# lia2790/walking-controllers

Measured on AMD Instinct MI355X. Metric: QP solves/sec (whole node), iCub IK-QP + DCM-MPC batch at 1/2/4/8 MI355X, higher is better.
Workload: dtype f64

## Files before the change

### include/wcqp.h

```cpp
#ifndef WCQP_H
#define WCQP_H

#include <stdint.h>

#ifdef __cplusplus
extern "C" {
#endif

#define WCQP_VERSION 400

#define WCQP_OK              0
#define WCQP_E_INVALID      (-1)
#define WCQP_E_UNSUPPORTED  (-2)
#define WCQP_E_NUMERIC      (-3)
#define WCQP_E_HIP          (-4)
#define WCQP_E_NOMEM        (-5)

#define WCQP_STATUS_SOLVED        0
#define WCQP_STATUS_MAX_ITER      1
#define WCQP_STATUS_INFEASIBLE    2
#define WCQP_STATUS_OUTSIDE_HULL  3
#define WCQP_STATUS_NUMERIC       4
#define WCQP_STATUS_STRUCTURE     5

// ... 101 lines not shown
                       double* foot_err, int32_t* iters);

typedef struct wcqp_qp_step {
    const double* x0; const double* ref; int32_t ref_len; const double* u_prev;
    const double* hull_A; const double* hull_b; const int32_t* hull_nc;
    double* u0; int32_t* mpc_status; uint32_t* mpc_active; double* mpc_margin; void* mpc_stream;
    const double* J_left; const double* J_right; const double* J_neck; const double* J_com;
    const double* q; const double* state;
    double* dq; int32_t* ik_status; uint32_t* active_lower; uint32_t* active_upper;
    double* foot_err; int32_t* iters; void* ik_stream;
} wcqp_qp_step;
int wcqp_qp_enqueue_steps(wcqp_mpc_t mpc, wcqp_ik_t ik, int32_t batch,
                          int32_t n_steps, const wcqp_qp_step* steps, int32_t* n_done);

#define WCQP_PLAN_WAYS_AUTO (-1)
typedef struct wcqp_qp_plan_s* wcqp_qp_plan_t;
int wcqp_qp_plan_create(wcqp_mpc_t mpc, wcqp_ik_t ik, int32_t batch, int32_t n_steps, const wcqp_qp_step* steps, int32_t ways,
                        wcqp_qp_plan_t* out);
int wcqp_qp_plan_enqueue(wcqp_qp_plan_t plan, void* stream);
int wcqp_qp_plan_destroy(wcqp_qp_plan_t plan);

#define WCQP_SLAB_IN_ARRAYS  12
#define WCQP_SLAB_OUT_ARRAYS 9
typedef struct wcqp_slab_layout {
    int32_t batch, ref_len;
    int64_t in_offset[WCQP_SLAB_IN_ARRAYS];
    int64_t in_bytes;
    int64_t out_offset[WCQP_SLAB_OUT_ARRAYS];
    int64_t out_bytes;
} wcqp_slab_layout;
int wcqp_slab_layout_for(int32_t batch, int32_t ref_len, wcqp_slab_layout* out);
int wcqp_qp_step_from_slabs(const wcqp_slab_layout* layout, const void* in_slab, void* out_slab, wcqp_qp_step* step);

#define WCQP_KIN_MAX_DOF 32
// ... 302 lines not shown
```

### walking-controllers_amd/capi.py

```python
from __future__ import annotations

import ctypes as C
import os
from typing import Optional

import numpy as np

_HERE = os.path.dirname(os.path.abspath(__file__))
LIB_PATH = os.environ.get("WCQP_LIB_PATH") or os.path.join(_HERE, "libwcqp.so")

VERSION = 400
WCQP_OK = OK = 0
E_INVALID, E_UNSUPPORTED, E_NUMERIC, E_HIP, E_NOMEM = -1, -2, -3, -4, -5
STATUS_SOLVED, STATUS_MAX_ITER, STATUS_INFEASIBLE, STATUS_OUTSIDE_HULL, STATUS_NUMERIC, STATUS_STRUCTURE = range(6)
IK_FORM_QPOASES, IK_FORM_OSQP = 0, 1
IK_ALG_DEFAULT, IK_ALG_SWEEP, IK_ALG_NULLSPACE, IK_ALG_NULLSPACE_MFMA, IK_ALG_NULLSPACE_16L, IK_ALG_BASE_ELIM = 0, 1, 2, 3, 4, 5
IK_JAC_AUTO, IK_JAC_MIXED, IK_JAC_GENERAL = 0, 1, 2
KIN_HANDOFF_NONE, KIN_HANDOFF_FUSED, KIN_HANDOFF_DENSE, KIN_HANDOFF_COMPACT = -1, 0, 1, 2
HULL_ROWS = 8
MAX_DOF = KIN_MAX_DOF = 32
IK_STATE_LEN = 87

ABI_SYMBOLS = (
    "wcqp_strerror", "wcqp_version", "wcqp_device_count", "wcqp_stream_create", "wcqp_stream_destroy", "wcqp_stream_synchronize",
    "wcqp_mpc_create", "wcqp_mpc_destroy", "wcqp_mpc_get_condensed", "wcqp_mpc_get_matrices",
    "wcqp_mpc_solve_device", "wcqp_mpc_solve_host",
    "wcqp_ik_create", "wcqp_ik_destroy", "wcqp_ik_set_posture", "wcqp_ik_solve_device", "wcqp_ik_solve_host",
    "wcqp_hull_from_feet_device", "wcqp_hull_from_feet_host",
    "wcqp_kin_create", "wcqp_kin_destroy", "wcqp_kin_jacobians_device", "wcqp_kin_jacobians_host",
    "wcqp_prepare_create", "wcqp_prepare_destroy", "wcqp_prepare_solve_device", "wcqp_prepare_solve_host",
    "wcqp_tick_create", "wcqp_tick_create_ext", "wcqp_tick_create_opts", "wcqp_tick_get_option", "wcqp_tick_get_info_ext", "wcqp_tick_destroy", "wcqp_tick_upload", "wcqp_tick_run", "wcqp_tick_download", "wcqp_tick_splice_reference",
    "wcqp_tick_set_feedback_device", "wcqp_tick_set_feedback_host", "wcqp_tick_get_info",
    "wcqp_tick_set_sensor_feedback_device", "wcqp_tick_set_sensor_feedback_host",
    "wcqp_tick_set_desired_device", "wcqp_tick_set_desired_host", "wcqp_tick_set_desired_from_plan",
    "wcqp_tick_upload_footsteps", "wcqp_tick_upload_footsteps_timed", "wcqp_tick_replan_footsteps_timed", "wcqp_tick_get_plan", "wcqp_tick_replan_footsteps", "wcqp_tick_replan_goals", "wcqp_tick_get_goal_result",
    "wcqp_tick_replan_goals_timed", "wcqp_tick_get_goal_timing",
    "wcqp_qp_enqueue_steps", "wcqp_qp_plan_create", "wcqp_qp_plan_enqueue", "wcqp_qp_plan_destroy",
    "wcqp_slab_layout_for", "wcqp_qp_step_from_slabs",
    "wcqp_unicycle_create", "wcqp_unicycle_destroy", "wcqp_unicycle_plan_device", "wcqp_unicycle_plan_host",
    "wcqp_unicycle_plan_timed_device", "wcqp_unicycle_plan_timed_host",
)


class WcqpError(RuntimeError):
    pass


class MpcParams(C.Structure):
    _fields_ = [("horizon", C.c_int32), ("sampling_time", C.c_double), ("com_height", C.c_double),
                ("gravity", C.c_double), ("Q", C.c_double * 4), ("R", C.c_double * 4),
                ("convex_hull_tolerance", C.c_double), ("feas_tol", C.c_double)]

# ... 66 lines not shown
class _Handle:

    def close(self):
        if self._h:
            getattr(lib(), self._destroy)(self._h)
            self._h = C.c_void_p()

    def __del__(self):
        try:
            self.close()
        except Exception:
            pass


PLAN_WAYS_AUTO = -1


class QpPlan(_Handle):
    _destroy = "wcqp_qp_plan_destroy"

    def __init__(self, mpc, ik, batch, steps, ways=1):
        self._h = C.c_void_p()
        self._keep = (mpc, ik, steps)
        check(lib().wcqp_qp_plan_create(mpc._h if mpc is not None else None, ik._h if ik is not None else None, int(batch), len(steps), steps, int(ways), C.byref(self._h)), "wcqp_qp_plan_create")

    def enqueue(self, stream=0):
        check(lib().wcqp_qp_plan_enqueue(self._h, stream or None), "wcqp_qp_plan_enqueue")


class KinParams(C.Structure):
    _fields_ = [("dof", C.c_int32), ("parent", C.c_int32 * 32),
                ("R0", (C.c_double * 9) * 32), ("p0", (C.c_double * 3) * 32), ("axis", (C.c_double * 3) * 32),
                ("mass", C.c_double * 32), ("com", (C.c_double * 3) * 32),
                ("root_mass", C.c_double), ("root_com", C.c_double * 3),
                ("frame_joint", C.c_int32 * 3), ("frame_R", (C.c_double * 9) * 3), ("frame_p", (C.c_double * 3) * 3)]


class PrepareParams(C.Structure):
    _fields_ = [("w_q", C.c_double), ("w_n", C.c_double), ("step_cap", C.c_double), ("tol_step", C.c_double), ("tol_constraint", C.c_double),
                ("max_iter", C.c_int32), ("q_reg", C.c_void_p), ("q_min", C.c_void_p), ("q_max", C.c_void_p)]


# ... 122 lines not shown


ABI_STRUCTS = {
    "wcqp_mpc_params": MpcParams, "wcqp_ik_params": IkParams, "wcqp_qp_step": QpStep, "wcqp_slab_layout": SlabLayout, "wcqp_kin_params": KinParams,
    "wcqp_prepare_params": PrepareParams, "wcqp_tick_params": TickParams, "wcqp_tick_params_ext": TickParamsExt, "wcqp_tick_option": TickOption,
    "wcqp_tick_inputs": TickInputs, "wcqp_tick_outputs": TickOutputs, "wcqp_tick_info": TickInfo, "wcqp_tick_info_ext": TickInfoExt,
    "wcqp_tick_desired": TickDesired, "wcqp_tick_footsteps": TickFootsteps, "wcqp_tick_replan": TickReplan, "wcqp_tick_plan_window": TickPlanWindow,
    "wcqp_tick_goals": TickGoals, "wcqp_tick_goal_result": TickGoalResult, "wcqp_tick_step_timing": TickStepTiming,
    "wcqp_unicycle_params": UnicycleParams, "wcqp_unicycle_inputs": UnicycleInputs, "wcqp_unicycle_outputs": UnicycleOutputs,
    "wcqp_unicycle_timing": UnicycleTiming,
}
ABI_CONSTANTS = {"WCQP_" + k: globals()[k] for k in (
    "VERSION OK E_INVALID E_UNSUPPORTED E_NUMERIC E_HIP E_NOMEM "
    "STATUS_SOLVED STATUS_MAX_ITER STATUS_INFEASIBLE STATUS_OUTSIDE_HULL STATUS_NUMERIC STATUS_STRUCTURE HULL_ROWS MAX_DOF IK_STATE_LEN "
    "IK_FORM_QPOASES IK_FORM_OSQP IK_ALG_DEFAULT IK_ALG_SWEEP IK_ALG_NULLSPACE IK_ALG_NULLSPACE_MFMA IK_ALG_NULLSPACE_16L IK_ALG_BASE_ELIM "
    "IK_JAC_AUTO IK_JAC_MIXED IK_JAC_GENERAL PLAN_WAYS_AUTO SLAB_IN_ARRAYS SLAB_OUT_ARRAYS KIN_MAX_DOF "
    "KIN_HANDOFF_FUSED KIN_HANDOFF_DENSE KIN_HANDOFF_COMPACT TICK_PLANT_INTERNAL TICK_PLANT_EXTERNAL TICK_DCM_MPC TICK_DCM_REACTIVE "
    "TICK_IK_VELOCITY TICK_IK_POSITION TICK_OPT_RESIDENT_PLAN TICK_OPT_POSITION_STREAMED TICK_OPT_PLAN_TIMED UNICYCLE_DONE UNICYCLE_TRUNCATED UNICYCLE_STUCK UNICYCLE_INVALID_INPUT "
    "TICK_MERGE_KEEP TICK_MERGE_AUTO TICK_SIDE_AUTO GOAL_KEPT GOAL_TOO_LATE").split()}

_lib: Optional[C.CDLL] = None


def lib() -> C.CDLL:
    global _lib
    if _lib is None:
        if not os.path.exists(LIB_PATH):
            raise WcqpError(f"{LIB_PATH} is missing: build it with __graft_entry__.build() "
                            "(make -C walking-controllers_amd/csrc); there is no fallback path")
        L = C.CDLL(LIB_PATH)
        dp, ip, up, vp = C.c_void_p, C.c_void_p, C.c_void_p, C.c_void_p
# ... 51 lines not shown
        L.wcqp_tick_replan_goals.argtypes = [C.c_void_p, C.c_void_p, C.POINTER(TickGoals), C.c_void_p]
        L.wcqp_tick_get_goal_result.argtypes = [C.c_void_p, C.POINTER(TickGoalResult)]
        L.wcqp_tick_replan_goals_timed.argtypes = [C.c_void_p, C.c_void_p, C.POINTER(UnicycleTiming), C.POINTER(TickGoals), C.c_void_p]
        L.wcqp_tick_get_goal_timing.argtypes = [C.c_void_p, C.c_void_p, C.c_void_p]
        L.wcqp_unicycle_create.argtypes = [C.POINTER(UnicycleParams), C.POINTER(C.c_void_p)]
        L.wcqp_unicycle_destroy.argtypes = [C.c_void_p]
        L.wcqp_unicycle_plan_device.argtypes = [C.c_void_p, C.c_int32, C.POINTER(UnicycleInputs), C.POINTER(UnicycleOutputs), C.c_void_p]
        L.wcqp_unicycle_plan_host.argtypes = [C.c_void_p, C.c_int32, C.POINTER(UnicycleInputs), C.POINTER(UnicycleOutputs)]
        L.wcqp_unicycle_plan_timed_device.argtypes = [C.c_void_p, C.POINTER(UnicycleTiming), C.c_int32, C.POINTER(UnicycleInputs), C.POINTER(UnicycleOutputs),
                                                      C.c_void_p, C.c_void_p, C.c_void_p]
        L.wcqp_unicycle_plan_timed_host.argtypes = [C.c_void_p, C.POINTER(UnicycleTiming), C.c_int32, C.POINTER(UnicycleInputs), C.POINTER(UnicycleOutputs),
                                                    C.c_void_p, C.c_void_p]
        L.wcqp_qp_enqueue_steps.argtypes = [C.c_void_p, C.c_void_p, C.c_int32, C.c_int32, C.POINTER(QpStep), C.POINTER(C.c_int32)]
        L.wcqp_qp_plan_create.argtypes = [C.c_void_p, C.c_void_p, C.c_int32, C.c_int32, C.POINTER(QpStep), C.c_int32, C.POINTER(C.c_void_p)]
        L.wcqp_qp_plan_enqueue.argtypes = [C.c_void_p, C.c_void_p]
        L.wcqp_qp_plan_destroy.argtypes = [C.c_void_p]
        L.wcqp_slab_layout_for.argtypes = [C.c_int32, C.c_int32, C.POINTER(SlabLayout)]
        L.wcqp_qp_step_from_slabs.argtypes = [C.POINTER(SlabLayout), C.c_void_p, C.c_void_p, C.POINTER(QpStep)]
        _lib = L
    return _lib


def check(rc: int, what: str = "wcqp call") -> None:
    if rc != WCQP_OK:
        raise WcqpError(f"{what} failed: {lib().wcqp_strerror(rc).decode()} ({rc})")


def _p(a: Optional[np.ndarray]):
    return None if a is None else a.ctypes.data_as(C.c_void_p)

# ... 712 lines not shown
```

### walking-controllers_amd/csrc/ik.hip

```cpp
#include <cmath>
#include <cstring>
#include <limits>
#include <new>
#include "ik_common.h"

using namespace wcqp_ik;
#ifdef WCQP_DIAG_KERNELS
#include "../../tools/diag/ik_sweep_kernel.h"
#endif

struct wcqp_ik_s {
    wcqp_ik_params p{};
    IkDeviceParams hp{};
    IkDeviceParams* d_prm = nullptr;
    wcqp::DeviceScratch scratch;
    wcqp::IkRoute route = wcqp::IkRoute::NULLSPACE_32;
    bool list_pass = false;
};

namespace {

int ensure_device(wcqp_ik_s* h) {
    if (h->d_prm) return WCQP_OK;
    if (const int rc = wcqp::require_device("IK solve path"); rc != WCQP_OK) return rc;
// ... 166 lines not shown
    if (!s.J_right || !s.J_neck || !s.J_com || !s.q || !s.state || !s.dq || !s.ik_status) return WCQP_E_INVALID;
    int rc = ensure_device(h);
    if (rc != WCQP_OK) return rc;
    rc = mpc_prepare(mpc);
    if (rc != WCQP_OK) return rc;
    wcqp_mpc::MpcDeviceConsts c;
    mpc_device_consts(mpc, &c);
    const wcqp_ik::IkIo io{s.J_left, s.J_right, s.J_neck, s.J_com, s.q, s.state, s.dq, s.ik_status, s.active_lower, s.active_upper, s.foot_err, s.iters};
    const hipStream_t st = (hipStream_t)s.ik_stream;
    rc = wcqp_ik::ik4_launch_pair(h->d_prm, batch, io, c, s.x0, s.ref, s.ref_len, s.u_prev, s.hull_A, s.hull_b, s.hull_nc,
                                  s.u0, s.mpc_status, s.mpc_active, s.mpc_margin, st);
    return rc != WCQP_OK || !h->list_pass ? rc : wcqp_ik::ik3_launch_list(h->d_prm, batch, io, st);
}
}

struct wcqp_qp_plan_s {
    wcqp_mpc_t mpc = nullptr;
    wcqp_ik_t ik = nullptr;
    int batch = 0, n_steps = 0, ways = 1;
    wcqp_qp_step* d_recs = nullptr;
    unsigned* d_queue = nullptr;
    int queue_grid = 0;
    bool mpc_only = false;
    bool ik_only = false;
};

extern "C" {

int wcqp_qp_plan_create(wcqp_mpc_t mpc, wcqp_ik_t ik, int32_t batch, int32_t n_steps, const wcqp_qp_step* steps, int32_t ways,
                        wcqp_qp_plan_t* out) {
    if (!out || batch < 1 || n_steps < 1 || !steps || ways < WCQP_PLAN_WAYS_AUTO) return WCQP_E_INVALID;
    if (ways == WCQP_PLAN_WAYS_AUTO) {
        const int groups = (batch + 3) / 4;
        ways = (16384 + groups - 1) / groups;
        if (ways < 4) ways = 4;
        if (ways > n_steps) ways = n_steps;
    }
    bool mpc_only = true;
    for (int k = 0; k < n_steps; ++k) mpc_only = mpc_only && !steps[k].J_left;
    bool ik_only = true;
// ... 15 lines not shown
    int rc = mpc_only ? WCQP_OK : ensure_device(ik);
    if (rc == WCQP_OK && mpc) rc = wcqp::mpc_prepare(mpc);
    if (rc != WCQP_OK) return rc;
    wcqp_qp_plan_s* p = new (std::nothrow) wcqp_qp_plan_s();
    if (!p) return WCQP_E_NOMEM;
    p->mpc = mpc; p->ik = mpc_only ? nullptr : ik; p->batch = batch; p->n_steps = n_steps; p->ways = ways < n_steps ? ways : n_steps;
    p->mpc_only = mpc_only; p->ik_only = ik_only;
    if (hipMalloc(reinterpret_cast<void**>(&p->d_recs), (size_t)n_steps * sizeof(wcqp_qp_step)) != hipSuccess) { delete p; return WCQP_E_NOMEM; }
    if (hipMemcpy(p->d_recs, steps, (size_t)n_steps * sizeof(wcqp_qp_step), hipMemcpyHostToDevice) != hipSuccess) {
        (void)hipFree(p->d_recs); delete p; return WCQP_E_HIP;
    }
    if (ways == 0) {
        p->queue_grid = wcqp_ik::ik4_plan_queue_grid(batch, n_steps);
        if (p->queue_grid < 1 || hipMalloc(reinterpret_cast<void**>(&p->d_queue), wcqp_ik::kPlanQueueBytes) != hipSuccess ||
            hipMemset(p->d_queue, 0, wcqp_ik::kPlanQueueBytes) != hipSuccess) {
            if (p->d_queue) (void)hipFree(p->d_queue);
            (void)hipFree(p->d_recs); delete p; return WCQP_E_HIP;
        }
        (void)hipStreamSynchronize(nullptr);
    }
    *out = p;
    return WCQP_OK;
}

int wcqp_qp_plan_enqueue(wcqp_qp_plan_t p, void* stream) {
    if (!p) return WCQP_E_INVALID;
    if (p->mpc_only) return wcqp::mpc_launch_plan(p->mpc, p->batch, p->d_recs, p->n_steps, p->ways, (hipStream_t)stream);
    wcqp_mpc::MpcDeviceConsts c{};
    if (p->mpc) wcqp::mpc_device_consts(p->mpc, &c);
    return wcqp_ik::ik4_launch_plan(p->ik->d_prm, p->batch, p->d_recs, p->n_steps, p->ways, c, (hipStream_t)stream, p->d_queue, p->queue_grid, p->ik_only);
}

int wcqp_qp_plan_destroy(wcqp_qp_plan_t p) {
    if (!p) return WCQP_E_INVALID;
    if (p->d_recs) (void)hipFree(p->d_recs);
    if (p->d_queue) (void)hipFree(p->d_queue);
    delete p;
    return WCQP_OK;
}

}

extern "C" {

int wcqp_ik_solve_host(wcqp_ik_t h, int32_t batch,
                       const double* J_left, const double* J_right, const double* J_neck, const double* J_com,
                       const double* q, const double* state,
                       double* dq, int32_t* status, uint32_t* active_lower, uint32_t* active_upper,
                       double* foot_err, int32_t* iters) {
    int rc = check_call(h, batch, J_left, J_right, J_neck, J_com, q, state, dq, status);
    if (rc != WCQP_OK || batch == 0) return rc;
    rc = ensure_device(h);
// ... 18 lines not shown
```

### walking-controllers_amd/csrc/ik4.hip

```cpp
#include "ik4_device.h"

namespace {

template <bool TICK, int JSRC, bool LOG = false, bool EXT = false>
__global__ __launch_bounds__(64, WCQP_IK4_WAVES)
void ik4_kernel(const IkDeviceParams* __restrict__ prm, int batch,
                const double* __restrict__ JL, const double* __restrict__ JR,
                const double* __restrict__ JN, const double* __restrict__ JC,
                const double* qpos, const double* __restrict__ state,
                double* __restrict__ dq_out, int* __restrict__ status_out,
                unsigned* __restrict__ alo_out, unsigned* __restrict__ aup_out,
                double* __restrict__ ferr_out, int* __restrict__ iters_out, const wcqp_tick::TickDev* __restrict__ tdp, int phase, int n_inner, int skip_last_mpc)
{
    __shared__ __attribute__((aligned(16))) double smem[4][PER_INST];
    if constexpr (TICK) {
        __shared__ __attribute__((aligned(16))) double kmodel[JSRC == 2 ? wcqp_tick::kKinTabSize : 2];
        __shared__ __attribute__((aligned(16))) double kgains[JSRC == 2 ? 4 * wcqp_tick::kGainsLdsStages : 2];
        ik4_tick_walk<JSRC, LOG, EXT, false>(prm, batch, JL, JR, JN, JC, qpos, state, dq_out, status_out, alo_out, aup_out, ferr_out, iters_out,
                                             tdp, phase, n_inner, skip_last_mpc, smem, kmodel, kgains);
    } else {
        ik4_body<TICK, JSRC>(prm, batch, JL, JR, JN, JC, qpos, state, dq_out, status_out, alo_out, aup_out, ferr_out, iters_out, wcqp_tick::TickDev{}, smem, xcd_group((int)blockIdx.x, (int)gridDim.x));
    }
}

// ... 71 lines not shown
            const unsigned u = (unsigned)__builtin_amdgcn_readfirstlane((int)k) * wcqp_ik::kPlanQueues + home;
            if (u < total) return u;
            home = (home + 1u) % wcqp_ik::kPlanQueues;
        }
        return total;
    };
    int r = (int)blockIdx.x / groups, blk = (int)blockIdx.x % groups;
#ifndef WCQP_PLAN_NO_XCD_MAP
    if ((groups & 7) == 0) {
        const int n = groups >> 3, x = (int)blockIdx.x & 7, k = (int)blockIdx.x >> 3;
        r = k / n; blk = x * n + k % n;
    }
#endif
    PlanTables pt;
    plan_tables_issue<TAB>(prm, c, WITH_MPC, ptab, pt);
    if (dynamic) {
        const unsigned u = draw();
        r = u < total ? (int)(u % (unsigned)n_steps) : n_steps; blk = u < total ? (int)(u / (unsigned)n_steps) : 0;
    }
#pragma unroll 1
    while (r < n_steps) {
        __asm__ volatile("" ::: "memory");
        using wcqp::as_global;
        const wcqp_qp_step& s = recs[r];
        MpcPairArgs m{c, WITH_MPC ? as_global(s.x0) : nullptr, WITH_MPC ? as_global(s.ref) : nullptr, s.ref_len, WITH_MPC ? as_global(s.u_prev) : nullptr,
                      WITH_MPC ? as_global(s.hull_A) : nullptr, WITH_MPC ? as_global(s.hull_b) : nullptr, WITH_MPC ? as_global(s.hull_nc) : nullptr,
                      WITH_MPC ? as_global(s.u0) : nullptr, WITH_MPC ? as_global(s.mpc_status) : nullptr, WITH_MPC ? as_global(s.mpc_active) : nullptr,
                      WITH_MPC ? as_global(s.mpc_margin) : nullptr,
                      dynamic ? queue + home * QS + z : nullptr, 0u, WITH_MPC};
        ik4_body<false, 0, true, false, false, false, false, false, TAB>(prm, batch, as_global(s.J_left), as_global(s.J_right), as_global(s.J_neck), as_global(s.J_com), as_global(s.q), as_global(s.state),
                                 as_global(s.dq), as_global(s.ik_status), as_global(s.active_lower), as_global(s.active_upper),
                                 as_global(s.foot_err), as_global(s.iters), wcqp_tick::TickDev{}, smem, blk, 0, true, nullptr, nullptr, &m, nullptr, nullptr, nullptr, &pt);
        wcqp::wave_lds_fence();
        pt.fill = false; pt.f_ik[0] = pt.f_ik[1] = pt.f_ik[2] = 0.0; pt.f_gr[0] = pt.f_gr[1] = make_double2(0.0, 0.0);
        if (dynamic) {
            unsigned u = (unsigned)__builtin_amdgcn_readfirstlane((int)m.ticket) * wcqp_ik::kPlanQueues + home;
            if (u >= total) { home = (home + 1u) % wcqp_ik::kPlanQueues; u = draw(); }
            r = u < total ? (int)(u % (unsigned)n_steps) : n_steps; blk = u < total ? (int)(u / (unsigned)n_steps) : 0;
        } else {
            r += ways;
        }
    }
    if (dynamic && threadIdx.x == 0) {
        __threadfence();
        if (atomicAdd(queue + wcqp_ik::kPlanQueues * QS, 1u) == gridDim.x - 1) {
            for (unsigned q = 0; q <= wcqp_ik::kPlanQueues; ++q) queue[q * QS] = 0u;
        }
    }
}
// ... 107 lines not shown
```

### walking-controllers_amd/csrc/ik4_device.h

```cpp
#pragma once
#include <cmath>
#include <cstddef>
#include <limits>
#include <type_traits>
#include "ik_common.h"
#include "tick_device.h"
#include "kin_device.h"
#include "ik4_layout.h"

namespace {

using wcqp_kin::st2;
using wcqp_kin::ld2;

struct MpcPairArgs {
    wcqp_mpc::MpcDeviceConsts c;
    const double* x0; const double* ref; int ref_len; const double* u_prev;
    const double* hull_A; const double* hull_b; const int* hull_nc;
    double* u0; int* status; unsigned* active; double* margin;
    unsigned* ticket_from = nullptr; unsigned ticket = 0;
    bool has_mpc = true;
};

#ifndef WCQP_PLAN_LDS
// ... 594 lines not shown
        {
            double* c = ct + j * LDC;
#pragma unroll
            for (int r = 0; r < NR; r += 2) st2(c + r, c0[r], c0[r + 1]);
            st2(c + NR, gt0, 0.0);
        }
        if (j < 8) {
            double* c = ct + col1 * LDC;
#pragma unroll
            for (int r = 0; r < NR; r += 2) st2(c + r, rhs1 ? 0.0 : c1[r], rhs1 ? 0.0 : c1[r + 1]);
            st2(c + NR, gt1, 0.0);
        }
        if (rhs1) {
#pragma unroll
            for (int r = 0; r < NR; r += 2) st2(dv + r, c1[r], c1[r + 1]);
            ct[24 * LDC] = 0.0; ct[24 * LDC + 1] = 0.0;
        }
    }
    wcqp::wave_lds_fence();
    WCQP_STAMP(10);
    {
        const int mk = lane & 15, mq = lane >> 4;
        v4d acc[4];
#pragma unroll
        for (int g = 0; g < 4; ++g) acc[g] = v4d{0.0, 0.0, 0.0, 0.0};
#pragma unroll
        for (int s = 0; s < 6; ++s) {
#pragma unroll
            for (int g = 0; g < 4; ++g) {
                const double v = smem[g][OFF_CT + (4 * s + mq) * LDC + mk];
                acc[g] = __builtin_amdgcn_mfma_f64_16x16x4f64(v, v, acc[g], 0, 0, 0);
// ... 775 lines not shown
```

### walking-controllers_amd/csrc/ik4_layout.h

```cpp
#pragma once
#include "ik_common.h"

namespace {

using namespace wcqp_ik;

typedef double v4d __attribute__((ext_vector_type(4)));

constexpr int NR = 12;
constexpr int NROWS_IN = 18;
constexpr int KMAX = kDof - 9;
constexpr int LDC = 14;

constexpr int OFF_ST = 0;
constexpr int OFF_BV = 112;
constexpr int OFF_DB = 130;
constexpr int OFF_CT = 0;
constexpr int OFF_PB = 0;
constexpr int A_SIZE = 340;
constexpr int OFF_COL = A_SIZE;
constexpr int OFF_YV = A_SIZE + 32;
constexpr int OFF_DV = A_SIZE + 48;
constexpr int OFF_YPV = A_SIZE;
constexpr int OFF_RV = A_SIZE + 16;
// ... 2 lines not shown
constexpr int PER_INST = 440;
constexpr int K_FS = 14, K_TW = 0, K_FRB = 322, K_FR = 358;
constexpr int K_MS = 394, K_MH = 410;
constexpr int K_PF = 434;
__host__ __device__ constexpr int k_sd(int m) { return K_TW + (16 + (m >> 1)) * K_FS + 12 + (m & 1); }
static_assert(K_MH + 24 <= K_PF && K_PF < PER_INST, "the flags stash is clear of the others");
static_assert(kDof * K_FS <= K_FRB && K_FR + 36 <= K_MS && K_MH + 24 <= PER_INST && k_sd(11) < kDof * K_FS && k_sd(0) >= 32 * 4, "kinematics scratch fits; the prefix sums [32][4] stay clear of the anchor pose");
static_assert(OFF_CT + 24 * LDC + 2 <= A_SIZE && OFF_DB + 18 <= A_SIZE && OFF_PB + 12 * 18 <= A_SIZE, "LDS overlays");
static_assert(OFF_ROWB + 16 <= PER_INST && OFF_DV + 16 <= PER_INST && (PER_INST % 32 == 24 || PER_INST % 32 == 8), "instances 16 banks apart");
static_assert(KMAX <= 24, "one slot index per C^T row");
static_assert(PER_INST * 8 * 4 * 11 <= 160 * 1024, "11 blocks per CU");

#ifndef WCQP_IK4_WAVES
#define WCQP_IK4_WAVES 2
#endif
#ifdef WCQP_IK_PLAN_VGPR_HALF
#define WCQP_IK_PLAN_REGS __attribute__((amdgpu_num_vgpr(WCQP_IK_PLAN_VGPR_HALF)))
#else
#define WCQP_IK_PLAN_REGS
#endif
#ifndef WCQP_IK4_KS
#define WCQP_IK4_KS 4
#endif

#define WCQP_STAMP_CLOCK(t__) asm volatile("s_memtime %0\n\ts_waitcnt lgkmcnt(0)" : "=s"(t__) :: "memory")
#define WCQP_STAMP_AT(k) do { if constexpr (TICK) { unsigned long long t__; WCQP_STAMP_CLOCK(t__); \
                                   if (lane == 0 && td.stamps) td.stamps[(size_t)blk * 16 + (k)] = t__; } } while (0)
#if defined(WCQP_TICK_KSTAMPS)
#define WCQP_STAMP(k) do { if constexpr ((k) == 0 || (k) == 12 || (k) == 14) WCQP_STAMP_AT(k); } while (0)
#define WCQP_KSTAMP(k) WCQP_STAMP_AT(k)
#elif defined(WCQP_TICK_STAMPS)
// ... 24 lines not shown
```

### walking-controllers_amd/csrc/mpc.hip

```cpp
#include <cmath>
#include <cstring>
#include <limits>
#include <new>
#include "wcqp_internal.h"
#include "mpc_device.h"

namespace {

using namespace wcqp_mpc;
constexpr int kBlock = 64;

__global__ __launch_bounds__(kBlock)
void mpc_condensed_kernel(MpcDeviceConsts c, int batch,
                          const double* __restrict__ x0, const double* __restrict__ ref, int ref_len,
                          int ref_stride, const int* __restrict__ ref_start,
                          const double* __restrict__ u_prev,
                          const double* __restrict__ hull_A, const double* __restrict__ hull_b,
                          const int* __restrict__ hull_nc, int hull_sets, const int* __restrict__ hull_sel,
                          double* __restrict__ u0_out, int* __restrict__ status_out,
                          unsigned* __restrict__ active_out, double* __restrict__ margin_out)
{
    __shared__ __attribute__((aligned(16))) double s_hull[kInstPerWave][WCQP_HULL_ROWS][4];

    const int lane = threadIdx.x;
// ... 6 lines not shown
    const int start = ref_start ? *ref_start : 0;
    const double2* rp = reinterpret_cast<const double2*>(ref) + inst * ref_stride + start;
    const long hset = inst * hull_sets + (hull_sel ? hull_sel[inst] : 0);
    double ux, uy, margin;
    int st;
    unsigned mask;
    mpc_row_solve(c, t, inst, x0, rp, ref_len, u_prev, hull_A, hull_b, hull_nc, hset, s_hull[sub], ux, uy, st, mask, margin);
    if (t == 0 && live) {
        reinterpret_cast<double2*>(u0_out)[inst] = make_double2(ux, uy);
        status_out[inst] = st;
        if (active_out) active_out[inst] = mask;
        if (margin_out) margin_out[inst] = margin;
    }
}

#ifdef WCQP_MPC_PLAN_VGPR_HALF
__attribute__((amdgpu_num_vgpr(WCQP_MPC_PLAN_VGPR_HALF)))
#endif
__global__ __launch_bounds__(kBlock, 6)
void mpc_plan_kernel(MpcDeviceConsts c, int batch, const wcqp_qp_step* __restrict__ recs, int n_steps, int ways, int groups)
{
    __shared__ __attribute__((aligned(16))) double s_hull[kInstPerWave][WCQP_HULL_ROWS][4];
    __shared__ __attribute__((aligned(16))) double s_gr[4 * kGrLdsStages];
    using wcqp::as_global;
    const int way = (int)blockIdx.x / groups, blk = (int)blockIdx.x % groups;
    const bool staged = c.N < kGrLdsStages;
    if (staged) {
        const double2* gp = reinterpret_cast<const double2*>(c.Gr.get());
        const unsigned last = 2u * (unsigned)c.N + 1u, e0 = threadIdx.x, e1 = threadIdx.x + 64u;
        const double2 f0 = gp[e0 < last ? e0 : last], f1 = gp[e1 < last ? e1 : last];
        double* g = s_gr + 2 * threadIdx.x;
        g[0] = f0.x; g[1] = f0.y; g[128] = f1.x; g[129] = f1.y;
        wcqp::wave_lds_fence();
    }
#pragma unroll 1
    for (int r = way; r < n_steps; r += ways) {
        __asm__ volatile("" ::: "memory");
        int lane = threadIdx.x;
        __asm__ volatile("" : "+v"(lane));
        const int sub = lane / kLanesPerInstance, t = lane % kLanesPerInstance;
        const long inst_raw = (long)blk * kInstPerWave + sub;
        const bool live = inst_raw < batch;
        const long inst = live ? inst_raw : (long)batch - 1;
        const wcqp_qp_step& s = recs[r];
        const double2* rp = reinterpret_cast<const double2*>(as_global(s.ref)) + inst * s.ref_len;
        double ux, uy, margin;
        int st;
        unsigned mask;
        if (staged) {
            MpcLoads L;
#pragma unroll
            for (int k = 0; k < 4; ++k) {
                const int i = t + k * kLanesPerInstance;
                const int ic = i <= c.N ? i : c.N;
                L.r[k] = rp[ic < s.ref_len ? ic : s.ref_len - 1];
            }
            double2 xs = make_double2(0.0, 0.0), up = xs, ha = xs;
            double hb = 0.0;
            if (t == 0) { xs = reinterpret_cast<const double2*>(as_global(s.x0))[inst]; up = reinterpret_cast<const double2*>(as_global(s.u_prev))[inst]; }
            const int nc = as_global(s.hull_nc)[inst];
            if (t < WCQP_HULL_ROWS) {
                ha = reinterpret_cast<const double2*>(as_global(s.hull_A))[inst * WCQP_HULL_ROWS + t];
                hb = as_global(s.hull_b)[inst * WCQP_HULL_ROWS + t];
            }
            double px, py;
            mpc_row_partial_lds(c, t, L, s_gr, px, py);
            if (t == 0) mpc_row_add_state(c, xs, up, px, py);
            mpc_row_finish(c, t, px, py, nc, ha.x, ha.y, hb, s_hull[sub], ux, uy, st, mask, margin);
        } else {
            mpc_row_solve(c, t, inst, as_global(s.x0), rp, s.ref_len, as_global(s.u_prev), as_global(s.hull_A), as_global(s.hull_b), as_global(s.hull_nc), inst,
                          s_hull[sub], ux, uy, st, mask, margin);
        }
        if (t == 0 && live) {
            reinterpret_cast<double2*>(as_global(s.u0))[inst] = make_double2(ux, uy);
            as_global(s.mpc_status)[inst] = st;
            if (s.mpc_active) as_global(s.mpc_active)[inst] = mask;
            if (s.mpc_margin) as_global(s.mpc_margin)[inst] = margin;
        }
        wcqp::wave_lds_fence();
    }
}

}

struct wcqp_mpc_s {
    wcqp_mpc_params p{};
    int N = 0, n = 0, nx = 0, nu = 0;
    double a = 0, b = 0;
    std::vector<double> P, Aeq, grad_sub;
    std::vector<double> Gr;
    double Gx[4]{}, Gu[4]{}, S0[4]{};
    double* d_Gr = nullptr;
    int device = -1;
    wcqp::DeviceScratch scratch;
// ... 113 lines not shown
    int rc = check_call(h, batch, x0, ref, ref_len, ref_stride, u_prev, hull_A, hull_b, hull_nc, hull_sets, u0, status);
    if (rc != WCQP_OK || batch == 0) return rc;
    rc = ensure_device(h);
    if (rc != WCQP_OK) return rc;
    MpcDeviceConsts c;
    mpc_device_consts(h, &c);
    const unsigned grid = (unsigned)((batch + kInstPerWave - 1) / kInstPerWave);
    hipLaunchKernelGGL(mpc_condensed_kernel, dim3(grid), dim3(kBlock), 0, stream,
                       c, batch, x0, ref, ref_len, ref_stride, ref_start_dev, u_prev, hull_A, hull_b, hull_nc, hull_sets, hull_sel,
                       u0, status, active, margin);
    WCQP_HIP_TRY(hipGetLastError());
    return WCQP_OK;
}

int mpc_prepare(wcqp_mpc_t h) { return h ? ensure_device(h) : WCQP_E_INVALID; }
int mpc_launch_plan(wcqp_mpc_t h, int batch, const wcqp_qp_step* d_recs, int n_steps, int ways, hipStream_t stream) {
    if (!h || !d_recs || batch < 1 || n_steps < 1 || ways < 1) return WCQP_E_INVALID;
    wcqp_mpc::MpcDeviceConsts c;
    mpc_device_consts(h, &c);
    const int groups = (batch + wcqp_mpc::kInstPerWave - 1) / wcqp_mpc::kInstPerWave;
    hipLaunchKernelGGL(mpc_plan_kernel, dim3((unsigned)(groups * ways)), dim3(kBlock), 0, stream, c, batch, d_recs, n_steps, ways, groups);
    WCQP_HIP_TRY(hipGetLastError());
    return WCQP_OK;
}
void mpc_device_consts(wcqp_mpc_t h, wcqp_mpc::MpcDeviceConsts* c) {
    c->Gr = h->d_Gr;
    std::memcpy(c->Gx, h->Gx, sizeof(c->Gx));
    std::memcpy(c->Gu, h->Gu, sizeof(c->Gu));
    std::memcpy(c->S0, h->S0, sizeof(c->S0));
    c->feas_tol = h->p.feas_tol;
// ... 86 lines not shown
```

### walking-controllers_amd/csrc/wcqp_internal.h

```cpp
#pragma once
#include <hip/hip_runtime.h>
#include <cstdint>
#include <cstdio>
#include <vector>
#include "wcqp.h"
#include "host_stage.h"

#define WCQP_HIP_TRY(expr)                                                         \
    do {                                                                           \
        hipError_t e__ = (expr);                                                   \
        if (e__ != hipSuccess) {                                                   \
            std::fprintf(stderr, "[wcqp] %s failed: %s (%s:%d)\n", #expr,          \
                         hipGetErrorString(e__), __FILE__, __LINE__);              \
            return WCQP_E_HIP;                                                     \
        }                                                                          \
    } while (0)

namespace wcqp_mpc { struct MpcDeviceConsts; }
namespace wcqp {
inline bool fits32(long long count, long long row_bytes) {
    return count >= 0 && row_bytes >= 0 && (row_bytes == 0 || count <= (1ll << 32) / row_bytes);
}
constexpr long long kRowBytesIkJacobian = 6 * 29 * 8;
inline bool mpc_batch_fits32(long long batch, long long ref_len) { return fits32(batch, ref_len * 16) && fits32(batch, WCQP_HULL_ROWS * 16); }
// ... 13 lines not shown
struct HostStage : StageLayout {
    int upload(DeviceScratch& block);
    int upload(void* block, size_t capacity);
    int download() const;
};

int require_device(const char* what);

int mpc_enqueue(wcqp_mpc_t h, int batch, const double* x0, const double* ref, int ref_len, int ref_stride,
                const int* ref_start_dev, const double* u_prev,
                const double* hull_A, const double* hull_b, const int* hull_nc, int hull_sets, const int* hull_sel,
                double* u0, int* status, unsigned* active, double* margin, hipStream_t stream);
int mpc_horizon(wcqp_mpc_t h);
int mpc_prepare(wcqp_mpc_t h);
int mpc_launch_plan(wcqp_mpc_t h, int batch, const wcqp_qp_step* d_recs, int n_steps, int ways, hipStream_t stream);
int ik_prepare(wcqp_ik_t h);
const void* ik_device_params(wcqp_ik_t h);
int qp_pair_enqueue(wcqp_mpc_t mpc, wcqp_ik_t ik, int batch, const wcqp_qp_step& s);
enum class IkRoute { BASE_ELIM, NULLSPACE_16L, NULLSPACE_32, NULLSPACE_32_MFMA, SWEEP };
IkRoute ik_route(wcqp_ik_t h);
void mpc_dynamics(wcqp_mpc_t h, double* a, double* b);
int kin_prepare(wcqp_kin_t h);
int hull_tables_from_state(int batch, const double* foot_rect_host, const double* state_dev, int state_len,
                           double* tab_A, double* tab_b, int* tab_nc, hipStream_t stream);
bool kin_compact_layout(wcqp_kin_t h, unsigned masks[3], int* stride, int* off_d);
bool kin_fused_tables(wcqp_kin_t h, std::vector<double>& tab, int* n_rounds);

#if defined(__HIPCC__)
__device__ __forceinline__ void wave_lds_fence() {
    __builtin_amdgcn_fence(__ATOMIC_RELEASE, "wavefront");
// ... 36 lines not shown
```

Measured before the change: 1.225 billion.

## Add split plan form running resident MPC kernel on side stream alongside IK

```diff
diff --git a/include/wcqp.h b/include/wcqp.h
--- a/include/wcqp.h
+++ b/include/wcqp.h
@@ -139,10 +139,14 @@
                           int32_t n_steps, const wcqp_qp_step* steps, int32_t* n_done);
 
 #define WCQP_PLAN_WAYS_AUTO (-1)
+#define WCQP_PLAN_FORM_FUSED 0
+#define WCQP_PLAN_FORM_SPLIT 1
+#define WCQP_PLAN_FORM_SPLIT_IK_FIRST 2
 typedef struct wcqp_qp_plan_s* wcqp_qp_plan_t;
 int wcqp_qp_plan_create(wcqp_mpc_t mpc, wcqp_ik_t ik, int32_t batch, int32_t n_steps, const wcqp_qp_step* steps, int32_t ways,
                         wcqp_qp_plan_t* out);
 int wcqp_qp_plan_enqueue(wcqp_qp_plan_t plan, void* stream);
+int wcqp_qp_plan_form(wcqp_qp_plan_t plan);
 int wcqp_qp_plan_destroy(wcqp_qp_plan_t plan);
 
 #define WCQP_SLAB_IN_ARRAYS  12
diff --git a/walking-controllers_amd/capi.py b/walking-controllers_amd/capi.py
--- a/walking-controllers_amd/capi.py
+++ b/walking-controllers_amd/capi.py
@@ -35,7 +35,7 @@
     "wcqp_tick_set_desired_device", "wcqp_tick_set_desired_host", "wcqp_tick_set_desired_from_plan",
     "wcqp_tick_upload_footsteps", "wcqp_tick_upload_footsteps_timed", "wcqp_tick_replan_footsteps_timed", "wcqp_tick_get_plan", "wcqp_tick_replan_footsteps", "wcqp_tick_replan_goals", "wcqp_tick_get_goal_result",
     "wcqp_tick_replan_goals_timed", "wcqp_tick_get_goal_timing",
-    "wcqp_qp_enqueue_steps", "wcqp_qp_plan_create", "wcqp_qp_plan_enqueue", "wcqp_qp_plan_destroy",
+    "wcqp_qp_enqueue_steps", "wcqp_qp_plan_create", "wcqp_qp_plan_enqueue", "wcqp_qp_plan_form", "wcqp_qp_plan_destroy",
     "wcqp_slab_layout_for", "wcqp_qp_step_from_slabs",
     "wcqp_unicycle_create", "wcqp_unicycle_destroy", "wcqp_unicycle_plan_device", "wcqp_unicycle_plan_host",
     "wcqp_unicycle_plan_timed_device", "wcqp_unicycle_plan_timed_host",
@@ -132,6 +132,7 @@
 
 
 PLAN_WAYS_AUTO = -1
+PLAN_FORM_FUSED, PLAN_FORM_SPLIT, PLAN_FORM_SPLIT_IK_FIRST = 0, 1, 2
 
 
 class QpPlan(_Handle):
@@ -144,6 +145,12 @@
 
     def enqueue(self, stream=0):
         check(lib().wcqp_qp_plan_enqueue(self._h, stream or None), "wcqp_qp_plan_enqueue")
+
+    def form(self):
+        form = lib().wcqp_qp_plan_form(self._h)
+        if form < 0:
+            check(form, "wcqp_qp_plan_form")
+        return form
 
 
 class KinParams(C.Structure):
@@ -296,7 +303,7 @@
     "VERSION OK E_INVALID E_UNSUPPORTED E_NUMERIC E_HIP E_NOMEM "
     "STATUS_SOLVED STATUS_MAX_ITER STATUS_INFEASIBLE STATUS_OUTSIDE_HULL STATUS_NUMERIC STATUS_STRUCTURE HULL_ROWS MAX_DOF IK_STATE_LEN "
     "IK_FORM_QPOASES IK_FORM_OSQP IK_ALG_DEFAULT IK_ALG_SWEEP IK_ALG_NULLSPACE IK_ALG_NULLSPACE_MFMA IK_ALG_NULLSPACE_16L IK_ALG_BASE_ELIM "
-    "IK_JAC_AUTO IK_JAC_MIXED IK_JAC_GENERAL PLAN_WAYS_AUTO SLAB_IN_ARRAYS SLAB_OUT_ARRAYS KIN_MAX_DOF "
+    "IK_JAC_AUTO IK_JAC_MIXED IK_JAC_GENERAL PLAN_WAYS_AUTO PLAN_FORM_FUSED PLAN_FORM_SPLIT PLAN_FORM_SPLIT_IK_FIRST SLAB_IN_ARRAYS SLAB_OUT_ARRAYS KIN_MAX_DOF "
     "KIN_HANDOFF_FUSED KIN_HANDOFF_DENSE KIN_HANDOFF_COMPACT TICK_PLANT_INTERNAL TICK_PLANT_EXTERNAL TICK_DCM_MPC TICK_DCM_REACTIVE "
     "TICK_IK_VELOCITY TICK_IK_POSITION TICK_OPT_RESIDENT_PLAN TICK_OPT_POSITION_STREAMED TICK_OPT_PLAN_TIMED UNICYCLE_DONE UNICYCLE_TRUNCATED UNICYCLE_STUCK UNICYCLE_INVALID_INPUT "
     "TICK_MERGE_KEEP TICK_MERGE_AUTO TICK_SIDE_AUTO GOAL_KEPT GOAL_TOO_LATE").split()}
@@ -378,6 +385,7 @@
         L.wcqp_qp_enqueue_steps.argtypes = [C.c_void_p, C.c_void_p, C.c_int32, C.c_int32, C.POINTER(QpStep), C.POINTER(C.c_int32)]
         L.wcqp_qp_plan_create.argtypes = [C.c_void_p, C.c_void_p, C.c_int32, C.c_int32, C.POINTER(QpStep), C.c_int32, C.POINTER(C.c_void_p)]
         L.wcqp_qp_plan_enqueue.argtypes = [C.c_void_p, C.c_void_p]
+        L.wcqp_qp_plan_form.argtypes = [C.c_void_p]
         L.wcqp_qp_plan_destroy.argtypes = [C.c_void_p]
         L.wcqp_slab_layout_for.argtypes = [C.c_int32, C.c_int32, C.POINTER(SlabLayout)]
         L.wcqp_qp_step_from_slabs.argtypes = [C.POINTER(SlabLayout), C.c_void_p, C.c_void_p, C.POINTER(QpStep)]
diff --git a/walking-controllers_amd/csrc/ik.hip b/walking-controllers_amd/csrc/ik.hip
--- a/walking-controllers_amd/csrc/ik.hip
+++ b/walking-controllers_amd/csrc/ik.hip
@@ -1,6 +1,9 @@
 #include <cmath>
+#include <cstdio>
+#include <cstdlib>
 #include <cstring>
 #include <limits>
+#include <mutex>
 #include <new>
 #include "ik_common.h"
 
@@ -204,6 +207,7 @@
 }
 }
 
+enum class PlanForm { FUSED = WCQP_PLAN_FORM_FUSED, SPLIT_MPC_FIRST = WCQP_PLAN_FORM_SPLIT, SPLIT_IK_FIRST = WCQP_PLAN_FORM_SPLIT_IK_FIRST, INVALID };
 struct wcqp_qp_plan_s {
     wcqp_mpc_t mpc = nullptr;
     wcqp_ik_t ik = nullptr;
@@ -213,7 +217,48 @@
     int queue_grid = 0;
     bool mpc_only = false;
     bool ik_only = false;
+    PlanForm form = PlanForm::FUSED;
+    int cus = 0;
+    hipStream_t side = nullptr;
+    hipEvent_t fork = nullptr, join = nullptr;
 };
+
+namespace {
+constexpr PlanForm kDefaultPlanForm = PlanForm::FUSED;
+PlanForm plan_form() {
+    const char* e = std::getenv("WCQP_PLAN_FORM");
+    if (!e || !*e) return kDefaultPlanForm;
+    if (!std::strcmp(e, "fused")) return PlanForm::FUSED;
+    if (!std::strcmp(e, "split")) return PlanForm::SPLIT_MPC_FIRST;
+    if (!std::strcmp(e, "split-ik-first")) return PlanForm::SPLIT_IK_FIRST;
+    std::fprintf(stderr, "[wcqp] WCQP_PLAN_FORM=%s: expected fused, split or split-ik-first\n", e);
+    return PlanForm::INVALID;
+}
+#ifndef WCQP_PLAN_EVENT_FLAGS
+#define WCQP_PLAN_EVENT_FLAGS hipEventDisableTiming
+#endif
+hipStream_t plan_side_stream(int dev) {
+    static std::mutex mu;
+    static hipStream_t streams[64] = {};
+    if (dev < 0 || dev >= 64) return nullptr;
+    std::lock_guard<std::mutex> lock(mu);
+    if (!streams[dev]) {
+        hipStream_t s = nullptr;
+        hipEvent_t e = nullptr;
+        if (hipStreamCreateWithFlags(&s, hipStreamNonBlocking) != hipSuccess) return nullptr;
+        if (hipEventCreateWithFlags(&e, hipEventDisableTiming) == hipSuccess) { (void)hipEventRecord(e, s); (void)hipStreamSynchronize(s); (void)hipEventDestroy(e); }
+        streams[dev] = s;
+    }
+    return streams[dev];
+}
+void plan_free(wcqp_qp_plan_s* p) {
+    if (p->d_recs) (void)hipFree(p->d_recs);
+    if (p->d_queue) (void)hipFree(p->d_queue);
+    if (p->fork) (void)hipEventDestroy(p->fork);
+    if (p->join) (void)hipEventDestroy(p->join);
+    delete p;
+}
+}
 
 extern "C" {
 
@@ -259,10 +304,22 @@
         p->queue_grid = wcqp_ik::ik4_plan_queue_grid(batch, n_steps);
         if (p->queue_grid < 1 || hipMalloc(reinterpret_cast<void**>(&p->d_queue), wcqp_ik::kPlanQueueBytes) != hipSuccess ||
             hipMemset(p->d_queue, 0, wcqp_ik::kPlanQueueBytes) != hipSuccess) {
-            if (p->d_queue) (void)hipFree(p->d_queue);
-            (void)hipFree(p->d_recs); delete p; return WCQP_E_HIP;
+            plan_free(p); return WCQP_E_HIP;
         }
         (void)hipStreamSynchronize(nullptr);
+    }
+    if (!mpc_only && !ik_only && ways > 0) {
+        p->form = plan_form();
+        if (p->form == PlanForm::INVALID) { plan_free(p); return WCQP_E_INVALID; }
+    }
+    if (p->form != PlanForm::FUSED) {
+        int dev = 0;
+        if (hipGetDevice(&dev) != hipSuccess || hipDeviceGetAttribute(&p->cus, hipDeviceAttributeMultiprocessorCount, dev) != hipSuccess || p->cus < 1 ||
+            !(p->side = plan_side_stream(dev)) ||
+            hipEventCreateWithFlags(&p->fork, WCQP_PLAN_EVENT_FLAGS) != hipSuccess ||
+            hipEventCreateWithFlags(&p->join, WCQP_PLAN_EVENT_FLAGS) != hipSuccess) {
+            plan_free(p); return WCQP_E_HIP;
+        }
     }
     *out = p;
     return WCQP_OK;
@@ -273,14 +330,25 @@
     if (p->mpc_only) return wcqp::mpc_launch_plan(p->mpc, p->batch, p->d_recs, p->n_steps, p->ways, (hipStream_t)stream);
     wcqp_mpc::MpcDeviceConsts c{};
     if (p->mpc) wcqp::mpc_device_consts(p->mpc, &c);
-    return wcqp_ik::ik4_launch_plan(p->ik->d_prm, p->batch, p->d_recs, p->n_steps, p->ways, c, (hipStream_t)stream, p->d_queue, p->queue_grid, p->ik_only);
-}
+    const hipStream_t st = (hipStream_t)stream;
+    if (p->form == PlanForm::FUSED)
+        return wcqp_ik::ik4_launch_plan(p->ik->d_prm, p->batch, p->d_recs, p->n_steps, p->ways, c, st, p->d_queue, p->queue_grid, p->ik_only);
+    WCQP_HIP_TRY(hipEventRecord(p->fork, st));
+    int rc = WCQP_OK;
+    if (p->form == PlanForm::SPLIT_IK_FIRST) rc = wcqp_ik::ik4_launch_plan(p->ik->d_prm, p->batch, p->d_recs, p->n_steps, p->ways, c, st, nullptr, 0,  true);
+    WCQP_HIP_TRY(hipStreamWaitEvent(p->side, p->fork, 0));
+    if (rc == WCQP_OK) rc = wcqp::mpc_launch_plan_resident(p->mpc, p->batch, p->d_recs, p->n_steps, p->cus, p->side);
+    if (rc == WCQP_OK && p->form == PlanForm::SPLIT_MPC_FIRST) rc = wcqp_ik::ik4_launch_plan(p->ik->d_prm, p->batch, p->d_recs, p->n_steps, p->ways, c, st, nullptr, 0,  true);
+    WCQP_HIP_TRY(hipEventRecord(p->join, p->side));
+    WCQP_HIP_TRY(hipStreamWaitEvent(st, p->join, 0));
+    return rc;
+}
+
+int wcqp_qp_plan_form(wcqp_qp_plan_t p) { return p ? (int)p->form : WCQP_E_INVALID; }
 
 int wcqp_qp_plan_destroy(wcqp_qp_plan_t p) {
     if (!p) return WCQP_E_INVALID;
-    if (p->d_recs) (void)hipFree(p->d_recs);
-    if (p->d_queue) (void)hipFree(p->d_queue);
-    delete p;
+    plan_free(p);
     return WCQP_OK;
 }
 
diff --git a/walking-controllers_amd/csrc/ik4.hip b/walking-controllers_amd/csrc/ik4.hip
--- a/walking-controllers_amd/csrc/ik4.hip
+++ b/walking-controllers_amd/csrc/ik4.hip
@@ -109,6 +109,9 @@
 #endif
     PlanTables pt;
     plan_tables_issue<TAB>(prm, c, WITH_MPC, ptab, pt);
+    if constexpr (!WITH_MPC) {
+        plan_tables_land<TAB>(pt, (int)threadIdx.x);
+    }
     if (dynamic) {
         const unsigned u = draw();
         r = u < total ? (int)(u % (unsigned)n_steps) : n_steps; blk = u < total ? (int)(u / (unsigned)n_steps) : 0;
@@ -116,6 +119,9 @@
 #pragma unroll 1
     while (r < n_steps) {
         __asm__ volatile("" ::: "memory");
+        if constexpr (!WITH_MPC) {
+            pt.fill = false; pt.f_ik[0] = pt.f_ik[1] = pt.f_ik[2] = 0.0; pt.f_gr[0] = pt.f_gr[1] = make_double2(0.0, 0.0);
+        }
         using wcqp::as_global;
         const wcqp_qp_step& s = recs[r];
         MpcPairArgs m{c, WITH_MPC ? as_global(s.x0) : nullptr, WITH_MPC ? as_global(s.ref) : nullptr, s.ref_len, WITH_MPC ? as_global(s.u_prev) : nullptr,
@@ -127,7 +133,7 @@
                                  as_global(s.dq), as_global(s.ik_status), as_global(s.active_lower), as_global(s.active_upper),
                                  as_global(s.foot_err), as_global(s.iters), wcqp_tick::TickDev{}, smem, blk, 0, true, nullptr, nullptr, &m, nullptr, nullptr, nullptr, &pt);
         wcqp::wave_lds_fence();
-        pt.fill = false; pt.f_ik[0] = pt.f_ik[1] = pt.f_ik[2] = 0.0; pt.f_gr[0] = pt.f_gr[1] = make_double2(0.0, 0.0);
+        if constexpr (WITH_MPC) { pt.fill = false; pt.f_ik[0] = pt.f_ik[1] = pt.f_ik[2] = 0.0; pt.f_gr[0] = pt.f_gr[1] = make_double2(0.0, 0.0); }
         if (dynamic) {
             unsigned u = (unsigned)__builtin_amdgcn_readfirstlane((int)m.ticket) * wcqp_ik::kPlanQueues + home;
             if (u >= total) { home = (home + 1u) % wcqp_ik::kPlanQueues; u = draw(); }
diff --git a/walking-controllers_amd/csrc/ik4_device.h b/walking-controllers_amd/csrc/ik4_device.h
--- a/walking-controllers_amd/csrc/ik4_device.h
+++ b/walking-controllers_amd/csrc/ik4_device.h
@@ -632,7 +632,9 @@
         if (rhs1) {
 #pragma unroll
             for (int r = 0; r < NR; r += 2) st2(dv + r, c1[r], c1[r + 1]);
-            ct[24 * LDC] = 0.0; ct[24 * LDC + 1] = 0.0;
+            double z = 0.0;
+            if constexpr (TAB == 2) __asm__ volatile("" : "+v"(z));
+            ct[24 * LDC] = z; ct[24 * LDC + 1] = z;
         }
     }
     wcqp::wave_lds_fence();
diff --git a/walking-controllers_amd/csrc/ik4_layout.h b/walking-controllers_amd/csrc/ik4_layout.h
--- a/walking-controllers_amd/csrc/ik4_layout.h
+++ b/walking-controllers_amd/csrc/ik4_layout.h
@@ -40,7 +40,10 @@
 #ifndef WCQP_IK4_WAVES
 #define WCQP_IK4_WAVES 2
 #endif
-#ifdef WCQP_IK_PLAN_VGPR_HALF
+#ifndef WCQP_IK_PLAN_VGPR_HALF
+#define WCQP_IK_PLAN_VGPR_HALF 108
+#endif
+#if WCQP_IK_PLAN_VGPR_HALF > 0
 #define WCQP_IK_PLAN_REGS __attribute__((amdgpu_num_vgpr(WCQP_IK_PLAN_VGPR_HALF)))
 #else
 #define WCQP_IK_PLAN_REGS
diff --git a/walking-controllers_amd/csrc/mpc.hip b/walking-controllers_amd/csrc/mpc.hip
--- a/walking-controllers_amd/csrc/mpc.hip
+++ b/walking-controllers_amd/csrc/mpc.hip
@@ -44,6 +44,66 @@
     }
 }
 
+__device__ __forceinline__
+void mpc_plan_record(const MpcDeviceConsts& c, int batch, const wcqp_qp_step& s, int blk, bool staged, int lane,
+                     double (*s_hull)[WCQP_HULL_ROWS][4], const double* s_gr)
+{
+    using wcqp::as_global;
+    const int sub = lane / kLanesPerInstance, t = lane % kLanesPerInstance;
+    const long inst_raw = (long)blk * kInstPerWave + sub;
+    const bool live = inst_raw < batch;
+    const long inst = live ? inst_raw : (long)batch - 1;
+    const double2* rp = reinterpret_cast<const double2*>(as_global(s.ref)) + inst * s.ref_len;
+    double ux, uy, margin;
+    int st;
+    unsigned mask;
+    if (staged) {
+        MpcLoads L;
+#pragma unroll
+        for (int k = 0; k < 4; ++k) {
+            const int i = t + k * kLanesPerInstance;
+            const int ic = i <= c.N ? i : c.N;
+            L.r[k] = rp[ic < s.ref_len ? ic : s.ref_len - 1];
+        }
+        double2 xs = make_double2(0.0, 0.0), up = xs, ha = xs;
+        double hb = 0.0;
+        if (t == 0) { xs = reinterpret_cast<const double2*>(as_global(s.x0))[inst]; up = reinterpret_cast<const double2*>(as_global(s.u_prev))[inst]; }
+        const int nc = as_global(s.hull_nc)[inst];
+        if (t < WCQP_HULL_ROWS) {
+            ha = reinterpret_cast<const double2*>(as_global(s.hull_A))[inst * WCQP_HULL_ROWS + t];
+            hb = as_global(s.hull_b)[inst * WCQP_HULL_ROWS + t];
+        }
+        double px, py;
+        mpc_row_partial_lds(c, t, L, s_gr, px, py);
+        if (t == 0) mpc_row_add_state(c, xs, up, px, py);
+        mpc_row_finish(c, t, px, py, nc, ha.x, ha.y, hb, s_hull[sub], ux, uy, st, mask, margin);
+    } else {
+        mpc_row_solve(c, t, inst, as_global(s.x0), rp, s.ref_len, as_global(s.u_prev), as_global(s.hull_A), as_global(s.hull_b), as_global(s.hull_nc), inst,
+                      s_hull[sub], ux, uy, st, mask, margin);
+    }
+    if (t == 0 && live) {
+        reinterpret_cast<double2*>(as_global(s.u0))[inst] = make_double2(ux, uy);
+        as_global(s.mpc_status)[inst] = st;
+        if (s.mpc_active) as_global(s.mpc_active)[inst] = mask;
+        if (s.mpc_margin) as_global(s.mpc_margin)[inst] = margin;
+    }
+    wcqp::wave_lds_fence();
+}
+
+__device__ __forceinline__ bool mpc_plan_stage_gains(const MpcDeviceConsts& c, unsigned wave_lane, double* s_gr)
+{
+    const bool staged = c.N < kGrLdsStages;
+    if (staged) {
+        const double2* gp = reinterpret_cast<const double2*>(c.Gr.get());
+        const unsigned last = 2u * (unsigned)c.N + 1u, e0 = wave_lane, e1 = wave_lane + 64u;
+        const double2 f0 = gp[e0 < last ? e0 : last], f1 = gp[e1 < last ? e1 : last];
+        double* g = s_gr + 2 * wave_lane;
+        g[0] = f0.x; g[1] = f0.y; g[128] = f1.x; g[129] = f1.y;
+        wcqp::wave_lds_fence();
+    }
+    return staged;
+}
+
 #ifdef WCQP_MPC_PLAN_VGPR_HALF
 __attribute__((amdgpu_num_vgpr(WCQP_MPC_PLAN_VGPR_HALF)))
 #endif
@@ -52,62 +112,33 @@
 {
     __shared__ __attribute__((aligned(16))) double s_hull[kInstPerWave][WCQP_HULL_ROWS][4];
     __shared__ __attribute__((aligned(16))) double s_gr[4 * kGrLdsStages];
-    using wcqp::as_global;
     const int way = (int)blockIdx.x / groups, blk = (int)blockIdx.x % groups;
-    const bool staged = c.N < kGrLdsStages;
-    if (staged) {
-        const double2* gp = reinterpret_cast<const double2*>(c.Gr.get());
-        const unsigned last = 2u * (unsigned)c.N + 1u, e0 = threadIdx.x, e1 = threadIdx.x + 64u;
-        const double2 f0 = gp[e0 < last ? e0 : last], f1 = gp[e1 < last ? e1 : last];
-        double* g = s_gr + 2 * threadIdx.x;
-        g[0] = f0.x; g[1] = f0.y; g[128] = f1.x; g[129] = f1.y;
-        wcqp::wave_lds_fence();
-    }
+    const bool staged = mpc_plan_stage_gains(c, threadIdx.x, s_gr);
 #pragma unroll 1
     for (int r = way; r < n_steps; r += ways) {
         __asm__ volatile("" ::: "memory");
         int lane = threadIdx.x;
         __asm__ volatile("" : "+v"(lane));
-        const int sub = lane / kLanesPerInstance, t = lane % kLanesPerInstance;
-        const long inst_raw = (long)blk * kInstPerWave + sub;
-        const bool live = inst_raw < batch;
-        const long inst = live ? inst_raw : (long)batch - 1;
-        const wcqp_qp_step& s = recs[r];
-        const double2* rp = reinterpret_cast<const double2*>(as_global(s.ref)) + inst * s.ref_len;
-        double ux, uy, margin;
-        int st;
-        unsigned mask;
-        if (staged) {
-            MpcLoads L;
-#pragma unroll
-            for (int k = 0; k < 4; ++k) {
-                const int i = t + k * kLanesPerInstance;
-                const int ic = i <= c.N ? i : c.N;
-                L.r[k] = rp[ic < s.ref_len ? ic : s.ref_len - 1];
-            }
-            double2 xs = make_double2(0.0, 0.0), up = xs, ha = xs;
-            double hb = 0.0;
-            if (t == 0) { xs = reinterpret_cast<const double2*>(as_global(s.x0))[inst]; up = reinterpret_cast<const double2*>(as_global(s.u_prev))[inst]; }
-            const int nc = as_global(s.hull_nc)[inst];
-            if (t < WCQP_HULL_ROWS) {
-                ha = reinterpret_cast<const double2*>(as_global(s.hull_A))[inst * WCQP_HULL_ROWS + t];
-                hb = as_global(s.hull_b)[inst * WCQP_HULL_ROWS + t];
-            }
-            double px, py;
-            mpc_row_partial_lds(c, t, L, s_gr, px, py);
-            if (t == 0) mpc_row_add_state(c, xs, up, px, py);
-            mpc_row_finish(c, t, px, py, nc, ha.x, ha.y, hb, s_hull[sub], ux, uy, st, mask, margin);
-        } else {
-            mpc_row_solve(c, t, inst, as_global(s.x0), rp, s.ref_len, as_global(s.u_prev), as_global(s.hull_A), as_global(s.hull_b), as_global(s.hull_nc), inst,
-                          s_hull[sub], ux, uy, st, mask, margin);
-        }
-        if (t == 0 && live) {
-            reinterpret_cast<double2*>(as_global(s.u0))[inst] = make_double2(ux, uy);
-            as_global(s.mpc_status)[inst] = st;
-            if (s.mpc_active) as_global(s.mpc_active)[inst] = mask;
-            if (s.mpc_margin) as_global(s.mpc_margin)[inst] = margin;
-        }
-        wcqp::wave_lds_fence();
+        mpc_plan_record(c, batch, recs[r], blk, staged, lane, s_hull, s_gr);
+    }
+}
+
+constexpr int kResidentWaves = 4, kResidentBlock = kResidentWaves * 64;
+__global__ __launch_bounds__(kResidentBlock) __attribute__((amdgpu_waves_per_eu(6, 6)))
+void mpc_plan_resident_kernel(MpcDeviceConsts c, int batch, const wcqp_qp_step* __restrict__ recs, int n_steps, int groups)
+{
+    __shared__ __attribute__((aligned(16))) double s_hull[kResidentWaves][kInstPerWave][WCQP_HULL_ROWS][4];
+    __shared__ __attribute__((aligned(16))) double s_gr[kResidentWaves][4 * kGrLdsStages];
+    const unsigned wv = (unsigned)__builtin_amdgcn_readfirstlane((int)(threadIdx.x >> 6)), wl = threadIdx.x & 63u;
+    const bool staged = mpc_plan_stage_gains(c, wl, s_gr[wv]);
+    const unsigned total = (unsigned)n_steps * (unsigned)groups, stride = gridDim.x * (unsigned)kResidentWaves;
+#pragma unroll 1
+    for (unsigned u = blockIdx.x * (unsigned)kResidentWaves + wv; u < total; u += stride) {
+        __asm__ volatile("" ::: "memory");
+        int lane = threadIdx.x;
+        __asm__ volatile("" : "+v"(lane));
+        lane &= 63;
+        mpc_plan_record(c, batch, recs[u / (unsigned)groups], (int)(u % (unsigned)groups), staged, lane, s_hull[wv], s_gr[wv]);
     }
 }
 
@@ -251,6 +282,16 @@
 }
 
 int mpc_prepare(wcqp_mpc_t h) { return h ? ensure_device(h) : WCQP_E_INVALID; }
+int mpc_launch_plan_resident(wcqp_mpc_t h, int batch, const wcqp_qp_step* d_recs, int n_steps, int cus, hipStream_t stream) {
+    if (!h || !d_recs || batch < 1 || n_steps < 1 || cus < 1) return WCQP_E_INVALID;
+    const int groups = (batch + wcqp_mpc::kInstPerWave - 1) / wcqp_mpc::kInstPerWave;
+    if ((long long)groups * n_steps >= (1ll << 31)) return WCQP_E_INVALID;
+    wcqp_mpc::MpcDeviceConsts c;
+    mpc_device_consts(h, &c);
+    hipLaunchKernelGGL(mpc_plan_resident_kernel, dim3((unsigned)cus), dim3(kResidentBlock), 0, stream, c, batch, d_recs, n_steps, groups);
+    WCQP_HIP_TRY(hipGetLastError());
+    return WCQP_OK;
+}
 int mpc_launch_plan(wcqp_mpc_t h, int batch, const wcqp_qp_step* d_recs, int n_steps, int ways, hipStream_t stream) {
     if (!h || !d_recs || batch < 1 || n_steps < 1 || ways < 1) return WCQP_E_INVALID;
     wcqp_mpc::MpcDeviceConsts c;
diff --git a/walking-controllers_amd/csrc/wcqp_internal.h b/walking-controllers_amd/csrc/wcqp_internal.h
--- a/walking-controllers_amd/csrc/wcqp_internal.h
+++ b/walking-controllers_amd/csrc/wcqp_internal.h
@@ -51,6 +51,7 @@
 int mpc_horizon(wcqp_mpc_t h);
 int mpc_prepare(wcqp_mpc_t h);
 int mpc_launch_plan(wcqp_mpc_t h, int batch, const wcqp_qp_step* d_recs, int n_steps, int ways, hipStream_t stream);
+int mpc_launch_plan_resident(wcqp_mpc_t h, int batch, const wcqp_qp_step* d_recs, int n_steps, int cus, hipStream_t stream);
 int ik_prepare(wcqp_ik_t h);
 const void* ik_device_params(wcqp_ik_t h);
 int qp_pair_enqueue(wcqp_mpc_t mpc, wcqp_ik_t ik, int batch, const wcqp_qp_step& s);
```

After: 1.223 billion. No clear change (-0.1%).
